# jiamiya/HOPE

Measured on AMD Instinct MI355X. Metric: parallel env steps/sec (full CarParking step incl. obs + RS search), higher is better.
Workload: dtype f64

## Files before the change

hope_amd/csrc/hope_internal.h:

```cpp
#pragma once
#include <hip/hip_runtime.h>
#include <stdint.h>
#include "hope_env.h"

namespace hope {

constexpr uint32_t STAGE_NO_BEAMS = 0x1000;
constexpr uint32_t STAGE_NO_MASK = 0x2000;
constexpr uint32_t STAGE_NO_CULL = 0x4000;
constexpr uint32_t STAGE_ONE_SCENE = 0x8000;

struct RsWord {
    double len[5];
    double Lm;
    int code;
    int n;
    double pad;
};
constexpr int RS_WORDS_PER_SCENE = 48;
constexpr int RS_LIST_MAX_SCENES = 1 << 24;
__host__ __device__ inline int rs_list_pack(int scene, int n_obst) { return (int)(((unsigned)scene << 8) | (unsigned)n_obst); }
__host__ __device__ inline int rs_list_scene(int entry) { return (int)((unsigned)entry >> 8); }
__host__ __device__ inline int rs_list_n_obst(int entry) { return (int)((unsigned)entry & 0xFFu); }
constexpr int RS_IN_WORDS = 14;
constexpr double RS_MAXC = 0.3327130214085973;
constexpr int RS_REC_HDR = 16;
constexpr int RS_REC_ORDER = 10;
constexpr int RS_REC_KEYS = RS_REC_HDR;
constexpr int RS_REC_WORDS = RS_REC_KEYS + RS_WORDS_PER_SCENE;
constexpr int RS_REC_SEGS = RS_REC_WORDS + 8 * RS_WORDS_PER_SCENE;
constexpr int RS_SEGW = 8, RS_SEG_F32 = 5 * RS_SEGW, RS_SEG_TABLE = RS_SEG_F32 + 5 * 2;
constexpr int RS_REC_DOUBLES = RS_REC_SEGS + RS_SEG_TABLE * RS_WORDS_PER_SCENE;

struct RsParams {
    int n, max_obst;
    int tile_cap;
    int max_queue;
    int slot_base, slot_dir;
    int obs_f64;
    int prio_front;
    const float4* obb;
    const float4* fverts;
    const float4* fbox;
    const uint8_t* eflag;
    const double* verts;
    const int32_t* n_obst;
    const double* scene_c;
    const double* state;
    const double* rs_in;
    const int32_t* rs_count;
    const int32_t* rs_list;
    double* rs_rec;
    int8_t* rs_word;
    void* rs_lengths;
    int32_t* surv_count;
    int2* surv_list;
};

struct DlpCases {
    int n_cases;
    const double* dest;
    const int32_t* cand_off;
    const double* cand;
    const int32_t* case_set;
    const int32_t* set_off;
    const double* set_verts;
};

struct StepCold {
    double* traj;
    int32_t* traj_len;
    int32_t* traj_valid;
    int32_t* layer_valid;
    const double* pool_verts;
    const double* pool_c;
    const int32_t* pool_nobst;
    const int32_t* pool_cls[2];
    int pool_cls_n[2];
    int32_t* cur_pool;
    uint32_t* episode;
    unsigned long long redraw_seed;
    DlpCases dlp;
    int32_t* pool_overflow;
    const uint8_t* slot_cls;
    float4* fverts;
    float4* fbox;
    uint8_t* eflag;
};

struct CwDev {
    unsigned long long* episodes;
    unsigned long long* successes;
    unsigned long long* folded_e;
    unsigned long long* folded_s;
    double* win_n;
    double* win_s;
    double* prob;
    double* pw;
};

constexpr int BEV_IMG = HOPE_IMG_SIZE;
constexpr int BEV_TRAJ_LEN = HOPE_TRAJ_RENDER_LEN;
constexpr int BEV_LAYER_ROWS = 512, BEV_LAYER_STRIDE = 128;
constexpr int BEV_DYN_DIM = 256;
constexpr size_t BEV_DYN_BYTES = (size_t)BEV_DYN_DIM * BEV_DYN_DIM;
constexpr int BEV_SCENE_INTS = 16 + (3 + BEV_TRAJ_LEN) * 16 + (2 + BEV_TRAJ_LEN) * 64;
struct BevParams {
    int n, max_obst;
    const double* verts;
    const int32_t* n_obst;
    const double* scene_c;
    const double* state;
    const double* traj;
    const int32_t* traj_len;
    int32_t* traj_valid;
    uint8_t* layer;
    uint8_t* dyn;
    int32_t* layer_valid;
    int32_t* legacy_list;
    int32_t* rebuild;
    int* scratch;
    const uint8_t* active;
    uint8_t* img;
    int debug;
};

struct LaunchTimer {
    virtual void begin(int kind, hipStream_t s) = 0;
    virtual void end(hipStream_t s) = 0;
};
hipError_t launch_rs_search(const RsParams& p, hipStream_t stream, LaunchTimer* timer);
hipError_t rs_prof_read(unsigned long long* out , int reset);
hipError_t rs_init_tables();
hipError_t rs_fstat_read(unsigned long long* out , int reset);
hipError_t rs_fdump_read(double* out );
hipError_t rs_log_read(int* out , int cap, int* n, int reset);
size_t rs_lds_bytes(int max_obst);
size_t rs_screen_lds_bytes(int max_obst);
size_t rs_rec_bytes_per_scene();
hipError_t launch_bev_image(const BevParams& p, hipStream_t stream, LaunchTimer* timer, hipStream_t side = nullptr, hipEvent_t ev_fork = nullptr,
                            hipEvent_t ev_join = nullptr);
size_t bev_lds_bytes(bool legacy);

}
```

hope_amd/csrc/hope_rs.hip:

```cpp
#include <stdlib.h>

#include "hope_dev.h"
#include "hope_internal.h"

namespace hope {

namespace {

constexpr double MAXC = RS_MAXC;
constexpr double RS_STEP = 0.1;
constexpr double MAX_LENGTH = 1000.0;
constexpr int NCAND = 46;

enum { TS = 0, TL = 1, TR = 2 };

__device__ __forceinline__ double py_mod(double v, double w) {
    double m = hm_fmod(v, w);
    if (m != 0) { if ((w < 0) != (m < 0)) m += w; } else m = copysign(0.0, w);
    return m;
}
__device__ __forceinline__ double rs_M(double theta) {
    double phi = py_mod(theta, 2.0 * PI);
    if (phi < -PI) phi += 2.0 * PI;
    if (phi > PI) phi -= 2.0 * PI;
// ... 347 lines not shown
        const double sp = (q == 1 || q == 2) ? -PHI : PHI;
        const double ssp = (q == 1 || q == 2) ? -sPHI : sPHI, csp = cPHI;
        double t = 0, u = 0, v = 0;
        bool ok = false;
        switch (g) {
            case 0: ok = (q == 0 || q == 2) && rs_SLS(sx, sy, sp, t, u, v); break;
            case 1: ok = rs_LSL(sx, sy, sp, ssp, csp, t, u, v); break;
            case 2: ok = rs_LSR(sx, sy, sp, ssp, csp, t, u, v); break;
            case 3: case 4: ok = rs_LRL(sx, sy, sp, ssp, csp, t, u, v); break;
            case 5: ok = rs_LRLRn(sx, sy, sp, ssp, csp, t, u, v); break;
            case 6: ok = rs_LRLRp(sx, sy, sp, ssp, csp, t, u, v); break;
            case 7: case 9: ok = rs_LRSL(sx, sy, sp, ssp, csp, t, u, v); break;
            case 8: case 10: ok = rs_LRSR(sx, sy, sp, ssp, csp, t, u, v); break;
            default: ok = rs_LRSLR(sx, sy, sp, ssp, csp, t, u, v); break;
        }
        ok = ok && live;
        int t0 = TL, t1 = TS, t2_ = TL, t3 = 0, t4 = 0, n = 3;
        double l0 = t, l1 = u, l2 = v, l3 = 0, l4 = 0;
        switch (g) {
            case 0: t0 = TS; t1 = TL; t2_ = TS; break;
            case 1: t0 = TL; t1 = TS; t2_ = TL; break;
            case 2: t0 = TL; t1 = TS; t2_ = TR; break;
            case 3: t0 = TL; t1 = TR; t2_ = TL; break;
            case 4: t0 = TL; t1 = TR; t2_ = TL; l0 = v; l2 = t; break;
            case 5: n = 4; t0 = TL; t1 = TR; t2_ = TL; t3 = TR; l2 = -u; l3 = v; break;
            case 6: n = 4; t0 = TL; t1 = TR; t2_ = TL; t3 = TR; l2 = u; l3 = v; break;
            case 7: n = 4; t0 = TL; t1 = TR; t2_ = TS; t3 = TL; l1 = -hp; l2 = u; l3 = v; break;
            case 8: n = 4; t0 = TL; t1 = TR; t2_ = TS; t3 = TR; l1 = -hp; l2 = u; l3 = v; break;
            case 9: n = 4; t0 = TL; t1 = TS; t2_ = TR; t3 = TL; l0 = v; l1 = u; l2 = -hp; l3 = t; break;
            case 10: n = 4; t0 = TR; t1 = TS; t2_ = TR; t3 = TL; l0 = v; l1 = u; l2 = -hp; l3 = t; break;
            default: n = 5; t0 = TL; t1 = TR; t2_ = TS; t3 = TL; t4 = TR; l1 = -hp; l2 = u; l3 = -hp; l4 = v; break;
        }
        if (q & 1) { l0 = -l0; l1 = -l1; l2 = -l2; l3 = -l3; l4 = -l4; }
        if (q & 2) { t0 = mirror_type(t0); t1 = mirror_type(t1); t2_ = mirror_type(t2_); t3 = mirror_type(t3); t4 = mirror_type(t4); }
        if (n < 4) { t3 = 0; l3 = 0; }
        if (n < 5) { t4 = 0; l4 = 0; }
        const int code = pack_types(t0, t1, t2_, t3, t4, n);
        double L = 0;
        L = L + fabs(l0); L = L + fabs(l1); L = L + fabs(l2);
        if (n > 3) L = L + fabs(l3);
        if (n > 4) L = L + fabs(l4);

        bool dup = false;
        if (g == 4 || g == 6) {
            const double a0 = (q & 2) ? quad_get<2>(p0) : quad_get<0>(p0), a1 = (q & 2) ? quad_get<2>(p1) : quad_get<0>(p1);
            const double a2 = (q & 2) ? quad_get<2>(p2) : quad_get<0>(p2), a3 = (q & 2) ? quad_get<2>(p3) : quad_get<0>(p3);
            const int ak = (q & 2) ? quad_get<2>((int)pk) : quad_get<0>((int)pk);
            const double b0 = (q & 2) ? quad_get<3>(p0) : quad_get<1>(p0), b1 = (q & 2) ? quad_get<3>(p1) : quad_get<1>(p1);
            const double b2 = (q & 2) ? quad_get<3>(p2) : quad_get<1>(p2), b3 = (q & 2) ? quad_get<3>(p3) : quad_get<1>(p3);
            const int bk = (q & 2) ? quad_get<3>((int)pk) : quad_get<1>((int)pk);
            dup = (ak && rs_dup(n, a0, a1, a2, a3, 0, l0, l1, l2, l3, l4)) || (bk && rs_dup(n, b0, b1, b2, b3, 0, l0, l1, l2, l3, l4));
        }
        bool kept = ok && !dup && !(L >= MAX_LENGTH) && !(q & 1);
        {
            const double e0 = (q & 2) ? quad_get<2>(l0) : quad_get<0>(l0), e1 = (q & 2) ? quad_get<2>(l1) : quad_get<0>(l1);
            const double e2 = (q & 2) ? quad_get<2>(l2) : quad_get<0>(l2), e3 = (q & 2) ? quad_get<2>(l3) : quad_get<0>(l3);
            const double e4 = (q & 2) ? quad_get<2>(l4) : quad_get<0>(l4);
            const int ek = (q & 2) ? quad_get<2>((int)kept) : quad_get<0>((int)kept);
            if (q & 1) kept = ok && !dup && !(ek && rs_dup(n, e0, e1, e2, e3, e4, l0, l1, l2, l3, l4)) && !(L >= MAX_LENGTH);
        }
        const double Lm = L / MAXC;
        if (live) rec[RS_REC_KEYS + 4 * g + q] = kept ? Lm : -1.0;
        if (kept) {
            RsWord* w = words + 4 * g + q;
            w->len[0] = l0; w->len[1] = l1; w->len[2] = l2; w->len[3] = l3; w->len[4] = l4;
            w->Lm = Lm; w->code = code; w->n = n;
        }
        p0 = l0; p1 = l1; p2 = l2; p3 = l3; pk = kept;
    }
}

__global__ __launch_bounds__(64) void k_rs_segs(RsParams p) {
    set_wave_prio(p.prio_front);
    __shared__ double keyl[8][RS_WORDS_PER_SCENE];
    __shared__ double prl[8][RS_WORDS_PER_SCENE];
    __shared__ unsigned char hidl[8][RS_WORDS_PER_SCENE];
    __shared__ unsigned char ordl[8][RS_WORDS_PER_SCENE];
    __shared__ int ntl[8];
    __shared__ double hdrl[8][8];
    const int lane = threadIdx.x, ls = lane >> 3, k0 = lane & 7;
    const int qi = blockIdx.x * 8 + ls;
    const int qs = qi < p.max_queue ? qi : p.max_queue - 1;
    const int entry = p.rs_list[qs];
    const int scene = rs_list_scene(entry);
    double* rec = p.rs_rec + (size_t)(p.slot_base + p.slot_dir * qs) * RS_REC_DOUBLES;
    const int count = *p.rs_count;
    if ((int)blockIdx.x * 8 >= count) return;
    const bool live = qi < count;
    double keyv[RS_WORDS_PER_SCENE / 8];
#pragma unroll
    for (int j = 0; j < RS_WORDS_PER_SCENE / 8; j++) keyv[j] = live ? rec[RS_REC_KEYS + 8 * j + k0] : -1.0;
    const double* in = p.rs_in + (size_t)qs * RS_IN_WORDS;
    double hdr = 0.0;
    int hdr_n = 0;
    if (k0 < 3) hdr = in[k0];
    else if (k0 < 7) hdr = in[k0];
    else hdr_n = rs_list_n_obst(entry);
    unsigned long long keptm = 0;
#pragma unroll
    for (int j = 0; j < RS_WORDS_PER_SCENE / 8; j++) {
        const double key = live ? keyv[j] : -1.0;
        keyl[ls][8 * j + k0] = key;
        keptm |= ((__ballot(key >= 0.0) >> (8 * ls)) & 0xffull) << (8 * j);
    }
    __syncthreads();
    if (live && k0 == 0) {
        double* pr = prl[ls];
        unsigned char* hid = hidl[ls];
        int hn = 0;
        for (unsigned long long m = keptm; m; m &= m - 1) {
            const int c = __ffsll((long long)m) - 1;
            const double pv = keyl[ls][c];
            int i = hn++;
            pr[i] = pv; hid[i] = (unsigned char)c;
            while (i) {
                const int parent = (i - 1) >> 1;
                if (pr[parent] < pr[i]) break;
                const double tp = pr[i]; pr[i] = pr[parent]; pr[parent] = tp;
                const unsigned char ti = hid[i]; hid[i] = hid[parent]; hid[parent] = ti;
                i = parent;
            }
        }
        const int n_kept = hn;
        int no = 0;
        double lmin = 0;
        while (hn > 0) {
            const double lm = pr[0];
            if (no == 0) lmin = lm;
            if (lm > 1.6 * lmin && no + 1 > 2) break;
            ordl[ls][no++] = hid[0];
            if (hn == 1) { hn = 0; break; }
            hn--;
            pr[0] = pr[hn]; hid[0] = hid[hn];
            int i = 0;
            for (;;) {
                const int l = (i << 1) + 1, r = (i + 1) << 1;
                int low = (l < hn && pr[l] < pr[i]) ? l : i;
                if (r < hn && pr[r] < pr[low]) low = r;
                if (low == i) break;
                const double tp = pr[i]; pr[i] = pr[low]; pr[low] = tp;
                const unsigned char ti = hid[i]; hid[i] = hid[low]; hid[low] = ti;
                i = low;
            }
        }
        ntl[ls] = no;
        ((int2*)rec)[1] = make_int2(n_kept, no);
    }
    if (live) {
        if (k0 < 7) rec[2 + k0] = hdr;
        else ((int2*)rec)[0] = make_int2(scene, hdr_n);
        hdrl[ls][k0] = hdr;
    }
    __syncthreads();
    if (!live) return;
    const int n_test = ntl[ls];
    const unsigned char* order = ordl[ls];
    const double q0w = hdrl[ls][2];
    double sq0, cq0;
    hm_sincos(q0w, &sq0, &cq0);
    const double fq0x = hdrl[ls][0] - hdrl[ls][3], fq0y = hdrl[ls][1] - hdrl[ls][5];
    for (int k = k0; k < n_test; k += 8) {
        const double* W = rec + RS_REC_WORDS + 8 * (int)order[k];
        double len[5];
#pragma unroll
        for (int i = 0; i < 5; i++) len[i] = W[i];
        const double w6 = W[6];
        const int code = __double2loint(w6), nseg = __double2hiint(w6);
        double* tb = rec + RS_REC_SEGS + RS_SEG_TABLE * k;
        double ox = 0, oy = 0, hy = 0;
#pragma unroll
        for (int i = 0; i < 5; i++) {
            if (i < nseg) {
                const int m = type_of(code, i);
                const double l = len[i];
                double s_oy, c_oy;
                hm_sincos(hy, &s_oy, &c_oy);
                double* sp_ = tb + RS_SEGW * i;
                sp_[0] = ox; sp_[1] = oy; sp_[2] = hy; sp_[3] = c_oy; sp_[4] = s_oy; sp_[5] = (double)m; sp_[6] = l;
                if (i == 0) sp_[7] = w6;
                {
// ... 506 lines not shown
    const double r0 = lane < RS_REC_HDR ? rec[lane] : 0.0;
    const double* tables = rec + RS_REC_SEGS;
    {
        typedef __attribute__((address_space(3))) void* lds_ptr;
        const double2* t2 = (const double2*)tables;
        __builtin_amdgcn_global_load_lds((const void*)(t2 + lane), (lds_ptr)tabs, 16, 0, 0);
        if (lane < 2 * RS_SEG_TABLE - WAVE) __builtin_amdgcn_global_load_lds((const void*)(t2 + WAVE + lane), (lds_ptr)(tabs + 2 * WAVE), 16, 0, 0);
        const float4* gfv = p.fverts + (size_t)scene * p.max_obst * 2;
        const float4* gfb = p.fbox + (size_t)scene * p.max_obst;
        const uint32_t* gfl = (const uint32_t*)(p.eflag + (size_t)scene * eflag_stride(p.max_obst));
        float4* lfv = (float4*)fv;
        for (int base = 0; base < 2 * n_obst; base += WAVE)
            if (base + lane < 2 * n_obst) __builtin_amdgcn_global_load_lds((const void*)(gfv + base + lane), (lds_ptr)(lfv + base), 16, 0, 0);
        for (int base = 0; base < n_obst; base += WAVE)
            if (base + lane < n_obst) __builtin_amdgcn_global_load_lds((const void*)(gfb + base + lane), (lds_ptr)(fbox + base), 16, 0, 0);
        for (int base = 0; 4 * base < n_obst; base += WAVE)
            if (4 * (base + lane) < n_obst) __builtin_amdgcn_global_load_lds((const void*)(gfl + base + lane), (lds_ptr)((uint32_t*)eflag + base), 4, 0, 0);
    }
    asm volatile("s_waitcnt vmcnt(0)" ::: "memory");
    const int n_paths = __builtin_amdgcn_readlane(__double2hiint(r0), 1);
    if (n_paths == 0) return;
    const float fxmax = (float)(readlane_d(r0, 6) - readlane_d(r0, 5)), fymax = (float)(readlane_d(r0, 8) - readlane_d(r0, 7));
    lsync();
    const unsigned long long condemned = screen_words<TIMING>(lane, n_paths, n_obst, tables, tabs, pq, cand, fv, fbox, eflag, fxmax, fymax, tsec);
    if (lane == 0) {
        ((unsigned long long*)rec)[9] = condemned;
        if (condemned != ((1ull << n_paths) - 1)) p.surv_list[atomicAdd(p.surv_count, 1)] = make_int2(qidx, entry);
    }
}

template <int OCC, bool TIMING, bool STATS, bool PRE = false>
__global__ __launch_bounds__(64, OCC) void k_rs_validate_f(RsParams p, int obs_f64) {
    extern __shared__ __attribute__((aligned(16))) double lds[];
    const int lane = threadIdx.x;
    if (!(obs_f64 & 0x10000)) __builtin_amdgcn_s_setprio(1);
    unsigned long long tsec[16] = {};
    const unsigned long long tstart_ = TIMING ? __builtin_readcyclecounter() : 0;
    RS_T0();
    const int b_ = (int)blockIdx.x;
    int qidx, entry;
    if (PRE) {
        const int2 sv = p.surv_list[b_];
        if (b_ >= *p.surv_count) return;
        qidx = sv.x; entry = sv.y;
    } else {
#ifdef HOPE_RS_3TRIPS
        const int count = *p.rs_count;
        if (b_ >= count) return;
        qidx = scene_of_block(b_, count);
        entry = p.rs_list[qidx];
#else
        qidx = scene_of_block(b_, p.max_queue);
        entry = p.rs_list[qidx];
        const int count = *p.rs_count;
        if (qidx >= count) return;
#endif
    }
    const int slot = p.slot_base + p.slot_dir * qidx;
#ifndef HOPE_RS_HDR
    const int scene = rs_list_scene(entry);
    const int n_obst = rs_list_n_obst(entry);
#endif
    float2* fv = (float2*)lds;
    float4* fbox = (float4*)(lds + 4 * p.tile_cap);
    double* scr = lds + 6 * p.tile_cap;
    double* segp = scr + RSB_SEG;
    double* qpd = scr + RSB_QPD;
    int* cand = (int*)(scr + RSB_WORDS_F);
    double* tabl = scr + RSB_TABF;
    unsigned char* qseg = (unsigned char*)(cand + ((p.tile_cap + 3) & ~3));
    unsigned char* eflag = qseg + RSB_QCAP;

    const double* rec = p.rs_rec + (size_t)slot * RS_REC_DOUBLES;
    const double r0 = lane < RS_REC_HDR ? rec[lane] : 0.0;
    const double* tables = rec + RS_REC_SEGS;
#ifdef HOPE_RS_3TRIPS
    if (__builtin_amdgcn_readlane(__double2hiint(r0), 1) == 0) return;
#endif
#ifdef HOPE_RS_HDR
    const int scene = __builtin_amdgcn_readlane(__double2loint(r0), 0);
    const int n_obst = __builtin_amdgcn_readlane(__double2hiint(r0), 0);
    (void)entry;
#endif
    double tb = lane < RS_SEG_TABLE ? tables[lane] : 0.0;
    if (!PRE) {
        typedef __attribute__((address_space(3))) void* lds_ptr;
        const double2* t2 = (const double2*)tables;
        __builtin_amdgcn_global_load_lds((const void*)(t2 + lane), (lds_ptr)qpd, 16, 0, 0);
        if (lane < 2 * RS_SEG_TABLE - WAVE) __builtin_amdgcn_global_load_lds((const void*)(t2 + WAVE + lane), (lds_ptr)(qpd + 2 * WAVE), 16, 0, 0);
    }
    {
        typedef __attribute__((address_space(3))) void* lds_ptr;
        const float4* gfv = p.fverts + (size_t)scene * p.max_obst * 2;
        const float4* gfb = p.fbox + (size_t)scene * p.max_obst;
        const uint32_t* gfl = (const uint32_t*)(p.eflag + (size_t)scene * eflag_stride(p.max_obst));
        float4* lfv = (float4*)fv;
        for (int base = 0; base < 2 * n_obst; base += WAVE)
            if (base + lane < 2 * n_obst) __builtin_amdgcn_global_load_lds((const void*)(gfv + base + lane), (lds_ptr)(lfv + base), 16, 0, 0);
        for (int base = 0; base < n_obst; base += WAVE)
            if (base + lane < n_obst) __builtin_amdgcn_global_load_lds((const void*)(gfb + base + lane), (lds_ptr)(fbox + base), 16, 0, 0);
        for (int base = 0; 4 * base < n_obst; base += WAVE)
            if (4 * (base + lane) < n_obst) __builtin_amdgcn_global_load_lds((const void*)(gfl + base + lane), (lds_ptr)((uint32_t*)eflag + base), 4, 0, 0);
    }
    const int n_paths = __builtin_amdgcn_readlane(__double2hiint(r0), 1);
    if (n_paths == 0) {
        asm volatile("s_waitcnt vmcnt(0)" ::: "memory");
        return;
    }
    const double* verts_g = p.verts + (size_t)scene * p.max_obst * 8;
    const float fxmin = 0.0f, fxmax = (float)(readlane_d(r0, 6) - readlane_d(r0, 5)), fymin = 0.0f, fymax = (float)(readlane_d(r0, 8) - readlane_d(r0, 7));
    const double step = RS_STEP * MAXC;
    bool tile_pending = true;
    int found = -1;
    double* bad1 = scr + RSB_BAD;
    if (lane < 6) bad1[lane] = INFINITY;
    lsync();
    RS_T(0);
    const bool paranoid = (obs_f64 & 0x2000) != 0;
    unsigned long long st_pass = 0, st_hit = 0, st_exact = 0, st_unc = 0, st_bad_hit = 0, st_bad_clear = 0, st_samples = 0;
    unsigned long long st_why[5] = {};
    unsigned long long condemned = 0;
    if (PRE) condemned = (unsigned long long)__double_as_longlong(readlane_d(r0, 9));
    else if (!(obs_f64 & 0x20000)) {
        asm volatile("s_waitcnt vmcnt(0)" ::: "memory");
        tile_pending = false;
        condemned = screen_words<TIMING>(lane, n_paths, n_obst, tables, qpd, (int*)tabl ,
                                         cand, fv, fbox, eflag, fxmax, fymax, tsec);
        if (TIMING) t0_ = __builtin_readcyclecounter();
    }
    else {
        asm volatile("s_waitcnt vmcnt(0)" ::: "memory");
        tile_pending = false;
    }
    const bool verify_screen = STATS && paranoid;
    const bool all_condemned = condemned == ((1ull << n_paths) - 1);
    unsigned long long st_scr_words = __popcll(condemned), st_scr_dead = all_condemned ? 1 : 0, st_scr_bad = 0;
    if (!all_condemned || verify_screen) {
        const double T0 = g_rs_steps[lane], T1 = g_rs_steps[WAVE + lane], T2 = g_rs_steps[2 * WAVE + lane], T3 = g_rs_steps[3 * WAVE + lane];
        tabl[lane] = T0; tabl[WAVE + lane] = T1; tabl[2 * WAVE + lane] = T2; tabl[3 * WAVE + lane] = T3;
        lsync();
    }
    for (int idx = 1; idx <= n_paths; idx++) {
        if (all_condemned && !verify_screen) break;
        const double tcur = tb;
        if (idx < n_paths && lane < RS_SEG_TABLE) tb = tables[RS_SEG_TABLE * idx + lane];
        const double len0 = readlane_d(tcur, 6), w6 = readlane_d(tcur, 7);
        const int code = __double2loint(w6), nseg = __double2hiint(w6);
        const int cls1 = type_of(code, 0) * 2 + (len0 > 0.0 ? 1 : 0);
        if (bad1[cls1] > 0.0 && fabs(len0) >= bad1[cls1]) continue;
        const bool screened = (condemned >> (idx - 1)) & 1;
        if (screened && !verify_screen) continue;
        bool invalid = false;
        if (lane < RS_SEG_TABLE) segp[lane] = tcur;
        if (TIMING) tsec[9] += 1;
        {
            double zero;
            asm volatile("v_mov_b64 %0, 0" : "=v"(zero));
            if (lane == 0) { qpd[0] = zero; qseg[0] = (unsigned char)__double2loint(zero); }
        }
        int nq = 1;
        lsync();
        RS_T(1);
        const int win = 128;
        int i = 0, t_off = 0;
        bool seg_open = false, finished = false;
        double pd = 0, ll = 0.0, lprev = 0.0, d = 0, l = 0;
        while (!invalid && (!finished || nq > 0)) {
            while (!finished && nq + WAVE + 1 <= win) {
                if (TIMING) tsec[10] += 1;
                if (!seg_open) {
                    l = uni_d(segp[RSB_SEGW * i + 6]);
                    d = uni_d(l > 0.0 ? step : -step);
                    pd = uni_d((i >= 1 && (lprev * l) > 0) ? -d - ll : d - ll);
                    lprev = l;
                    seg_open = true;
                }
                double mine, t = pd;
                int ncap;
                if (i == 0 && t_off + WAVE <= RS_TAB) {
                    const double v = tabl[t_off + lane];
                    mine = d > 0.0 ? v : -v;
                    ncap = WAVE;
                    t_off += WAVE;
                    if (t_off < RS_TAB) {
                        const double nx = tabl[t_off];
                        t = d > 0.0 ? nx : -nx;
                    } else t = readlane_d(mine, WAVE - 1) + d;
                } else {
                    mine = pd;
                    double last = pd;
                    ncap = 0;
                    for (int j0 = 0; j0 < WAVE; j0 += 8) {
                        if ((lane >> 3) == (j0 >> 3)) mine = t;
#pragma unroll
                        for (int jj = 0; jj < 7; jj++) t = t + d;
                        last = t;
                        t = t + d;
                        ncap = j0 + 8;
                        if (__any(fabs(last) > fabs(l))) break;
                    }
#pragma unroll
                    for (int k = 0; k < 7; k++)
                        if (k < (lane & 7)) mine = mine + d;
                }
                const bool in_seg = lane < ncap && fabs(mine) <= fabs(l);
                const unsigned long long valid = (ncap == WAVE) ? ~0ull : ((1ull << ncap) - 1);
                const unsigned long long fail = ~__ballot(in_seg) & valid;
                const int cnt = fail ? (__ffsll((long long)fail) - 1) : ncap;
                if (lane < cnt) { qpd[nq + lane] = mine; qseg[nq + lane] = (unsigned char)i; }
                nq += cnt;
                if (fail) {
                    pd = readlane_d(mine, cnt);
                    ll = uni_d(l - pd - d);
                    seg_open = false;
                    if (i == nseg - 1) {
                        if (lane == 0) { qpd[nq] = l; qseg[nq] = (unsigned char)i; }
                        nq += 1;
                        finished = true;
                    }
                    i++;
                } else pd = uni_d(t);
            }
            lsync();
            RS_T(2);
            if (finished && segp[3 * RSB_SEGW + 7] != 0.0) nq = pop_trailing_zero_x(nq, segp, RSB_SEGW, qpd, qseg, lane);
            const int n_all = nq;
            const int n = finished ? n_all : (n_all & ~(WAVE - 1));
            const int stride = (n + WAVE - 1) >> 6;
            const int n_coarse = stride == 1 ? n : (stride == 2 ? (n + 1) >> 1 : ((n + 2) * 171) >> 9);
            const int n_rest = n - n_coarse;
            for (int rnd = 0; rnd == 0 || (rnd - 1) * WAVE < n_rest; rnd++) {
                int sidx;
                if (rnd == 0) sidx = (lane < n_coarse) ? stride * lane : -1;
                else { const int r = (rnd - 1) * WAVE + lane; sidx = r < n_rest ? r + (stride == 2 ? r : r >> 1) + 1 : -1; }
                const bool active = sidx >= 0;
                if (TIMING) tsec[11] += 1;
                float X = 0, Y = 0, hc = 1, hs = 0;
                int sg0 = 0;
                if (active) {
                    const float lf = (float)qpd[sidx];
                    sg0 = (int)qseg[sidx];
                    const float4 row = ((const float4*)(segp + RS_SEG_F32))[sg0];
                    const int m = type_of(code, sg0);
                    const float rev = lf * 0.15915494309189535f;
                    const float sl = m == TS ? 0.0f : __builtin_amdgcn_sinf(rev), cl = m == TS ? 1.0f : __builtin_amdgcn_cosf(rev);
                    const float sgn = m == TR ? -1.0f : 1.0f;
                    const float ldx = m == TS ? lf * F_INV_MAXC : sl * F_INV_MAXC;
                    const float ldy = sgn * (1.0f - cl) * F_INV_MAXC;
                    X = row.x + (row.z * ldx - row.w * ldy);
                    Y = row.y + (row.w * ldx + row.z * ldy);
                    const float ss = sgn * sl;
                    hc = row.z * cl - row.w * ss;
                    hs = row.w * cl + row.z * ss;
                }
                RS_T(3);
                int why_cnt = 0, hit_rec = -1;
                int ua = -1, ub = -1;
                bool uover = false;
                bool hit = active && (X < fxmin - FEPS || X > fxmax + FEPS || Y < fymin - FEPS || Y > fymax + FEPS);
                bool unc = active && !hit && (X < fxmin + FEPS || X > fxmax - FEPS || Y < fymin + FEPS || Y > fymax - FEPS);
                const float cx = X + hc * F_MID, cy = Y + hs * F_MID;
                const float ex = fabsf(hc) * F_HL + fabsf(hs) * F_HW + FEPS, ey = fabsf(hs) * F_HL + fabsf(hc) * F_HW + FEPS;
                const float lox = cx - ex, hix = cx + ex, loy = cy - ey, hiy = cy + ey;
                const float ulox = wave_min_f(active ? lox : INFINITY), uhix = wave_max_f(active ? hix : -INFINITY);
                const float uloy = wave_min_f(active ? loy : INFINITY), uhiy = wave_max_f(active ? hiy : -INFINITY);
                if (tile_pending) {
                    asm volatile("s_waitcnt vmcnt(0)" ::: "memory");
                    tile_pending = false;
                }
                int nc = 0;
                for (int base = 0; base < n_obst; base += WAVE) {
                    const int o = base + lane;
                    bool near = false;
                    if (o < n_obst) {
                        const float4 bb = fbox[o];
                        near = !(bb.x > uhix || bb.y < ulox || bb.z > uhiy || bb.w < uloy);
                    }
                    const unsigned long long mm = __ballot(near);
                    if (near) cand[nc + __popcll(mm & ((1ull << lane) - 1))] = o;
                    nc += __popcll(mm);
                }
                RS_T(4);
                if (nc > 0 && !__any(hit)) {
                    if (TIMING) { tsec[12] += 1; tsec[13] += nc; }
                    lsync();
                    const bool hull_ok = fminf(fabsf(hc), fabsf(hs)) >= FETA_HULL;
// ... 49 lines not shown
                            const bool certain = cross && corners_ok && angle_ok && hull_ok && ((efl >> k) & 1);
                            const bool mine_open = (open >> k) & 1;
                            if (mine_open && certain) { hit = true; if (STATS && hit_rec < 0) hit_rec = r * 4 + k; }
                            if (STATS && mine_open && !certain) why_cnt |= 1 << (!cross ? 0 : !((efl >> k) & 1) ? 1 : !hull_ok ? 2 : !corners_ok ? 3 : 4);
                            if (!__any(hit) && mine_open && !certain) {
                                unc = true;
                                if (ua < 0) ua = r | (0x100 << k);
                                else if ((ua & 0xff) == r) ua |= 0x100 << k;
                                else if (ub < 0) ub = r | (0x100 << k);
                                else if ((ub & 0xff) == r) ub |= 0x100 << k;
                                else uover = true;
                            }
                        }
                        if (__any(hit)) break;
                    }
                    lsync();
                }
                RS_T(5);
                bool bad = hit;
                const bool any_hit = __any(hit);
                const bool need64 = (STATS && paranoid) || (!any_hit && __any(unc));
                (void)need64;
                if (STATS) {
                    st_pass += 1;
                    if (any_hit) st_hit += 1;
                    if (!any_hit && __any(unc)) {
                        const unsigned long long wm = __ballot(why_cnt != 0);
                        int wor = 0;
                        for (int b = 0; b < 5; b++) if (__any((why_cnt >> b) & 1)) wor |= 1 << b;
                        for (int b = 0; b < 5; b++) st_why[b] += (wor >> b) & 1;
                        (void)wm;
                    }
                }
                if (STATS && paranoid) {
                    const double q0x = rec[2], q0y = rec[3], q0w = rec[4], xmin = rec[5], xmax = rec[6], ymin = rec[7], ymax = rec[8];
                    const double c_q = rec[RS_REC_SEGS + RS_SEGW + 7], s_q = rec[RS_REC_SEGS + 2 * RS_SEGW + 7];
                    const bool ex = exact_pass<true>(active ? sidx : -1, segp, qpd, qseg, c_q, s_q, q0x, q0y, q0w, verts_g, p.obb + (size_t)scene * p.max_obst, cand, n_obst, xmin, xmax, ymin, ymax, lane);
                    st_samples += __popcll(__ballot(active));
                    st_bad_hit += __popcll(__ballot(active && hit && !ex));
                    if (active && ((hit && !ex) || (!any_hit && !hit && !unc && ex))) {
                        const int di = (int)atomicAdd(&g_rs_fstat[15], 1ull);
                        if (di < 64) {
                            double px = 0, py = 0, pyaw = 0;
                            const double spd = qpd[sidx];
                            const double* sp_ = segp + RSB_SEGW * (int)qseg[sidx];
                            interpolate(spd, (int)sp_[5], sp_[0], sp_[1], sp_[2], sp_[3], -sp_[4], sp_[3], sp_[4], px, py, pyaw);
                            const double wyaw = pi_2_pi(pyaw + q0w);
                            double* dd = g_rs_fdump + 16 * di;
                            dd[0] = scene; dd[1] = idx; dd[2] = spd; dd[3] = (double)qseg[sidx]; dd[4] = X; dd[5] = Y; dd[6] = hc; dd[7] = hs;
                            dd[8] = c_q * px + s_q * py; dd[9] = -s_q * px + c_q * py; dd[10] = hm_cos(wyaw); dd[11] = hm_sin(wyaw);
                            dd[12] = hit ? 1.0 : 0.0; dd[13] = (double)why_cnt; dd[14] = sp_[5]; dd[15] = (double)hit_rec;
                        }
                    }
                    if (!any_hit) st_bad_clear += __popcll(__ballot(active && !hit && !unc && ex));
                    bad = ex;
                } else if (!any_hit && __any(unc)) {
                    if (STATS) { st_exact += 1; st_unc += __popcll(__ballot(unc)); }
                    bad = exact_edges(unc, sidx, ua, ub, uover, cand, nc, segp, qpd, qseg, verts_g, rec);
                }
                if (TIMING) t0_ = __builtin_readcyclecounter();
                if (__any(bad)) {
                    const double mine1 = (bad && active && qseg[sidx] == 0) ? fabs(qpd[sidx]) : INFINITY;
                    const double v = fmin(bad1[cls1], wave_min_d(mine1));
                    lsync();
                    if (lane < 6 && (lane == cls1 || v == 0.0)) bad1[lane] = fmin(bad1[lane], v);
                    invalid = true;
                    break;
                }
            }
            {
                const int rem = n_all - n;
                double cd = 0;
                unsigned char cs = 0;
                if (lane < rem) { cd = qpd[n + lane]; cs = qseg[n + lane]; }
                lsync();
                if (lane < rem) { qpd[lane] = cd; qseg[lane] = cs; }
                nq = rem;
            }
            lsync();
        }
        if (STATS && screened && !invalid) { st_scr_bad += 1; continue; }
        if (!invalid) { found = idx - 1; break; }
    }
    if (STATS && lane == 0) {
        atomicAdd(&g_rs_fstat[7], st_scr_bad); atomicAdd(&g_rs_fstat[13], st_scr_words); atomicAdd(&g_rs_fstat[14], st_scr_dead);
        for (int b = 0; b < 5; b++) atomicAdd(&g_rs_fstat[8 + b], st_why[b]);
        atomicAdd(&g_rs_fstat[0], st_pass); atomicAdd(&g_rs_fstat[1], st_hit); atomicAdd(&g_rs_fstat[2], st_exact);
        atomicAdd(&g_rs_fstat[3], st_unc); atomicAdd(&g_rs_fstat[4], st_bad_hit); atomicAdd(&g_rs_fstat[5], st_bad_clear);
        atomicAdd(&g_rs_fstat[6], st_samples);
    }
    if (TIMING) {
        tsec[6] = __builtin_readcyclecounter() - tstart_;
        tsec[8] = 1;
        if (lane == 0) {
            for (int i = 0; i < 16; i++) if (tsec[i]) atomicAdd(&g_rs_prof[(blockIdx.x & 63) * 16 + i], tsec[i]);
            const int li = atomicAdd(&g_rs_log_n, 1);
            if (li < RS_LOG_CAP) g_rs_log[li] = make_int4((int)tsec[6], (int)tsec[9] | (n_paths << 8) | ((p.tile_cap > 32) << 16), (int)tsec[11], found >= 0);
        }
    }
    if (found < 0) return;
    const double wlen = lane < 5 ? segp[RSB_SEGW * lane + 6] : 0.0;
    const int code = __double2loint(segp[7]), nseg = __double2hiint(segp[7]);
    if (lane < 5) {
        double lm = lane < nseg ? wlen / MAXC : 0.0;
        if (p.rs_lengths) {
            if (obs_f64 & 1) ((double*)p.rs_lengths)[5 * (size_t)scene + lane] = lm;
            else ((float*)p.rs_lengths)[5 * (size_t)scene + lane] = (float)lm;
        }
        p.rs_word[8 * (size_t)scene + lane] = lane < nseg ? (int8_t)type_of(code, lane) : (int8_t)HOPE_RS_NONE;
    }
    if (lane == 5) p.rs_word[8 * (size_t)scene + 5] = (int8_t)nseg;
    if (lane == 6) p.rs_word[8 * (size_t)scene + 6] = 1;
}

}

static size_t rs_lds_bytes_exact(int max_obst) {
    return (size_t)(10 * max_obst + RSB_WORDS) * 8 + (size_t)((max_obst + 3) & ~3) * 4 + RSB_QCAP;
}
static size_t rs_lds_bytes_filter(int max_obst) {
    return (size_t)(6 * max_obst + RSB_WORDS_F) * 8 + (size_t)((max_obst + 3) & ~3) * 4 + RSB_QCAP + (size_t)((max_obst + 3) & ~3);
}
size_t rs_lds_bytes(int max_obst) { return std::max(rs_lds_bytes_exact(max_obst), rs_lds_bytes_filter(max_obst)); }
size_t rs_screen_lds_bytes(int max_obst) {
    return (size_t)(6 * max_obst + 4 * RS_SEG_TABLE) * 8 + 2 * WAVE * 4 + (size_t)((max_obst + 3) & ~3) * 4 + (size_t)((max_obst + 3) & ~3);
}
size_t rs_rec_bytes_per_scene() { return sizeof(double) * RS_REC_DOUBLES; }

hipError_t rs_prof_read(unsigned long long* out, int reset) {
    hipError_t e = hipDeviceSynchronize();
    if (e != hipSuccess) return e;
    static unsigned long long buf[64 * 16];
    e = hipMemcpyFromSymbol(buf, HIP_SYMBOL(g_rs_prof), sizeof(buf));
    for (int i = 0; i < 16; i++) { out[i] = 0; for (int sh = 0; sh < 64; sh++) out[i] += buf[sh * 16 + i]; }
    if (e == hipSuccess && reset) {
        for (auto& v : buf) v = 0;
        e = hipMemcpyToSymbol(HIP_SYMBOL(g_rs_prof), buf, sizeof(buf));
    }
    return e;
}

hipError_t rs_fdump_read(double* out ) {
    hipError_t e = hipDeviceSynchronize();
    if (e != hipSuccess) return e;
    return hipMemcpyFromSymbol(out, HIP_SYMBOL(g_rs_fdump), sizeof(double) * 64 * 16);
}

hipError_t rs_log_read(int* out , int cap, int* n, int reset) {
    hipError_t e = hipDeviceSynchronize();
    if (e != hipSuccess) return e;
    e = hipMemcpyFromSymbol(n, HIP_SYMBOL(g_rs_log_n), sizeof(int));
    if (e != hipSuccess) return e;
    const int m = *n < cap ? (*n < RS_LOG_CAP ? *n : RS_LOG_CAP) : cap;
    if (m > 0) e = hipMemcpyFromSymbol(out, HIP_SYMBOL(g_rs_log), sizeof(int4) * (size_t)m);
    if (e == hipSuccess && reset) { const int z = 0; e = hipMemcpyToSymbol(HIP_SYMBOL(g_rs_log_n), &z, sizeof(int)); }
    return e;
}

hipError_t rs_fstat_read(unsigned long long* out , int reset) {
    hipError_t e = hipDeviceSynchronize();
    if (e != hipSuccess) return e;
    e = hipMemcpyFromSymbol(out, HIP_SYMBOL(g_rs_fstat), 16 * sizeof(unsigned long long));
    if (e == hipSuccess && reset) {
        unsigned long long z[16] = {};
        e = hipMemcpyToSymbol(HIP_SYMBOL(g_rs_fstat), z, sizeof(z));
    }
    return e;
}

hipError_t rs_init_tables() {
    static bool done[64] = {};
    int dev = 0;
    hipError_t e = hipGetDevice(&dev);
    if (e != hipSuccess) return e;
    if (dev >= 0 && dev < 64 && done[dev]) return hipSuccess;
    double tab[RS_TAB];
    const volatile double step = RS_STEP * MAXC;
    volatile double t = step;
    for (int k = 0; k < RS_TAB; k++) { tab[k] = t; t = t + step; }
    e = hipMemcpyToSymbol(HIP_SYMBOL(g_rs_steps), tab, sizeof(tab));
    if (e == hipSuccess && dev >= 0 && dev < 64) done[dev] = true;
    return e;
}

constexpr int RS_LARGE_TILE_WPC = 6;
constexpr int RS_PRIO_MIN_SCENES = 32768;

hipError_t launch_rs_search(const RsParams& p, hipStream_t stream, LaunchTimer* timer) {
    if (p.max_queue <= 0) return hipSuccess;
    static const bool timing = getenv("HOPE_RS_TIMING") != nullptr;
    const bool exact = getenv("HOPE_RS_EXACT") != nullptr;
    const int dbg = getenv("HOPE_RS_DEBUG") ? (int)strtol(getenv("HOPE_RS_DEBUG"), nullptr, 0) : 0;
    const bool stats = (dbg & 0x6000) != 0;
    size_t lds = exact ? rs_lds_bytes_exact(p.tile_cap) : rs_lds_bytes_filter(p.tile_cap);
    if (!exact && p.tile_cap > 32) lds = std::max(lds, (size_t)((158 * 1024 / RS_LARGE_TILE_WPC) & ~255));
    if (lds > 48 * 1024) {
        hipError_t e = hipFuncSetAttribute((const void*)k_rs_validate_f<RSF_OCC, false, false, true>, hipFuncAttributeMaxDynamicSharedMemorySize, (int)lds);
        if (e != hipSuccess) return e;
    }
    const void* vk = exact ? (timing ? (const void*)k_rs_validate<3, true> : (const void*)k_rs_validate<3, false>)
                           : (timing ? (const void*)k_rs_validate_f<RSF_OCC, true, false> : stats ? (const void*)k_rs_validate_f<RSF_OCC, false, true>
                              : (const void*)k_rs_validate_f<RSF_OCC, false, false>);
    if (lds > 48 * 1024) {
        hipError_t e = hipFuncSetAttribute(vk, hipFuncAttributeMaxDynamicSharedMemorySize, (int)lds);
        if (e != hipSuccess) return e;
    }
    if (!exact) { hipError_t e = rs_init_tables(); if (e != hipSuccess) return e; }
    if (timer) timer->begin(HOPE_K_RS_WORDS, stream);
    hipLaunchKernelGGL(k_rs_words, dim3((p.max_queue + RSA_SCENES - 1) / RSA_SCENES, RSA_GROUPS), dim3(WAVE), 0, stream, p);
    if (timer) timer->end(stream);
    if (timer) timer->begin(HOPE_K_RS_SEGS, stream);
    hipLaunchKernelGGL(k_rs_segs, dim3((p.max_queue + 7) / 8), dim3(WAVE), 0, stream, p);
    if (timer) timer->end(stream);
    const bool split = !exact && !timing && !stats && !(dbg & 0x20000) && p.surv_count && p.surv_list &&
                       getenv("HOPE_RS_SPLIT") && atoi(getenv("HOPE_RS_SPLIT")) == 1;
    if (split) {
        if (timer) timer->begin(HOPE_K_RS_SCREEN, stream);
        hipLaunchKernelGGL((k_rs_screen<false, 8>), dim3(p.max_queue), dim3(WAVE), rs_screen_lds_bytes(p.tile_cap), stream, p);
        if (timer) timer->end(stream);
    }
    if (timer) timer->begin(HOPE_K_RS_VALIDATE, stream);
    const bool longer_chain = 2 * (long long)p.max_queue >= p.n;
    const int flags = (p.obs_f64 ? 1 : 0) | dbg | ((p.n < RS_PRIO_MIN_SCENES || !longer_chain) ? 0x10000 : 0);
    if (exact) {
        if (timing) hipLaunchKernelGGL((k_rs_validate<3, true>), dim3(p.max_queue), dim3(WAVE), lds, stream, p, flags);
        else hipLaunchKernelGGL((k_rs_validate<3, false>), dim3(p.max_queue), dim3(WAVE), lds, stream, p, flags);
    } else if (split) hipLaunchKernelGGL((k_rs_validate_f<RSF_OCC, false, false, true>), dim3(p.max_queue), dim3(WAVE), lds, stream, p, flags);
    else if (timing) hipLaunchKernelGGL((k_rs_validate_f<RSF_OCC, true, false>), dim3(p.max_queue), dim3(WAVE), lds, stream, p, flags);
    else if (stats) hipLaunchKernelGGL((k_rs_validate_f<RSF_OCC, false, true>), dim3(p.max_queue), dim3(WAVE), lds, stream, p, flags);
    else hipLaunchKernelGGL((k_rs_validate_f<RSF_OCC, false, false>), dim3(p.max_queue), dim3(WAVE), lds, stream, p, flags);
    if (timer) timer->end(stream);
    return hipGetLastError();
}

}
```

Measured before the change: 162.0 million.

## Async-load RS step table into LDS and skip condemned words in validate

The validate kernel now iterates only over non-condemned candidate words using a bitmask instead of scanning every index. It stages the step table into LDS with asynchronous global_load_lds, waiting on vmcnt only when the table is first needed. The segs kernel issues its key and input loads before the early-exit check to overlap latency. An optional env-gated path syncs the stream to shrink the validate grid to the live count.

```diff
diff --git a/hope_amd/csrc/hope_internal.h b/hope_amd/csrc/hope_internal.h
--- a/hope_amd/csrc/hope_internal.h
+++ b/hope_amd/csrc/hope_internal.h
@@ -55,6 +55,7 @@
     void* rs_lengths;
     int32_t* surv_count;
     int2* surv_list;
+    const double* rs_steps = nullptr;
 };
 
 struct DlpCases {
@@ -131,7 +132,7 @@
 };
 hipError_t launch_rs_search(const RsParams& p, hipStream_t stream, LaunchTimer* timer);
 hipError_t rs_prof_read(unsigned long long* out , int reset);
-hipError_t rs_init_tables();
+hipError_t rs_init_tables(const double** steps = nullptr);
 hipError_t rs_fstat_read(unsigned long long* out , int reset);
 hipError_t rs_fdump_read(double* out );
 hipError_t rs_log_read(int* out , int cap, int* n, int reset);
diff --git a/hope_amd/csrc/hope_rs.hip b/hope_amd/csrc/hope_rs.hip
--- a/hope_amd/csrc/hope_rs.hip
+++ b/hope_amd/csrc/hope_rs.hip
@@ -453,20 +453,18 @@
     const int qi = blockIdx.x * 8 + ls;
     const int qs = qi < p.max_queue ? qi : p.max_queue - 1;
     const int entry = p.rs_list[qs];
-    const int scene = rs_list_scene(entry);
     double* rec = p.rs_rec + (size_t)(p.slot_base + p.slot_dir * qs) * RS_REC_DOUBLES;
+    double keyv[RS_WORDS_PER_SCENE / 8];
+#pragma unroll
+    for (int j = 0; j < RS_WORDS_PER_SCENE / 8; j++) keyv[j] = rec[RS_REC_KEYS + 8 * j + k0];
+    const double* in = p.rs_in + (size_t)qs * RS_IN_WORDS;
+    const double hdr_in = in[k0 < 7 ? k0 : 0];
     const int count = *p.rs_count;
     if ((int)blockIdx.x * 8 >= count) return;
     const bool live = qi < count;
-    double keyv[RS_WORDS_PER_SCENE / 8];
-#pragma unroll
-    for (int j = 0; j < RS_WORDS_PER_SCENE / 8; j++) keyv[j] = live ? rec[RS_REC_KEYS + 8 * j + k0] : -1.0;
-    const double* in = p.rs_in + (size_t)qs * RS_IN_WORDS;
-    double hdr = 0.0;
-    int hdr_n = 0;
-    if (k0 < 3) hdr = in[k0];
-    else if (k0 < 7) hdr = in[k0];
-    else hdr_n = rs_list_n_obst(entry);
+    const int scene = rs_list_scene(entry);
+    const double hdr = k0 < 7 ? hdr_in : 0.0;
+    const int hdr_n = k0 < 7 ? 0 : rs_list_n_obst(entry);
     unsigned long long keptm = 0;
 #pragma unroll
     for (int j = 0; j < RS_WORDS_PER_SCENE / 8; j++) {
@@ -1139,8 +1137,9 @@
     const int n_obst = __builtin_amdgcn_readlane(__double2hiint(r0), 0);
     (void)entry;
 #endif
-    double tb = lane < RS_SEG_TABLE ? tables[lane] : 0.0;
-    if (!PRE) {
+    double tb = 0.0;
+    if (PRE) { if (lane < RS_SEG_TABLE) tb = tables[lane]; }
+    else {
         typedef __attribute__((address_space(3))) void* lds_ptr;
         const double2* t2 = (const double2*)tables;
         __builtin_amdgcn_global_load_lds((const void*)(t2 + lane), (lds_ptr)qpd, 16, 0, 0);
@@ -1192,21 +1191,33 @@
     const bool verify_screen = STATS && paranoid;
     const bool all_condemned = condemned == ((1ull << n_paths) - 1);
     unsigned long long st_scr_words = __popcll(condemned), st_scr_dead = all_condemned ? 1 : 0, st_scr_bad = 0;
-    if (!all_condemned || verify_screen) {
-        const double T0 = g_rs_steps[lane], T1 = g_rs_steps[WAVE + lane], T2 = g_rs_steps[2 * WAVE + lane], T3 = g_rs_steps[3 * WAVE + lane];
-        tabl[lane] = T0; tabl[WAVE + lane] = T1; tabl[2 * WAVE + lane] = T2; tabl[3 * WAVE + lane] = T3;
+    unsigned long long todo = verify_screen ? (1ull << n_paths) - 1 : ((1ull << n_paths) - 1) & ~condemned;
+    bool tab_ready = false;
+    if (todo) {
+        const int k = __ffsll((long long)todo) - 1;
+        const int lk = PRE ? -1 : k - ((obs_f64 & 0x20000) ? 0 : ((n_paths - 1) & ~3));
+        if (!PRE && lk >= 0) { if (lane < RS_SEG_TABLE) tb = qpd[RS_SEG_TABLE * lk + lane]; }
+        else if (!PRE || k > 0) { if (lane < RS_SEG_TABLE) tb = tables[RS_SEG_TABLE * k + lane]; }
+        typedef __attribute__((address_space(3))) void* lds_ptr;
+        const double2* s2 = (const double2*)p.rs_steps;
         lsync();
-    }
-    for (int idx = 1; idx <= n_paths; idx++) {
-        if (all_condemned && !verify_screen) break;
+        __builtin_amdgcn_global_load_lds((const void*)(s2 + lane), (lds_ptr)tabl, 16, 0, 0);
+        __builtin_amdgcn_global_load_lds((const void*)(s2 + WAVE + lane), (lds_ptr)(tabl + 2 * WAVE), 16, 0, 0);
+    }
+    for (bool first_word = true; todo; first_word = false) {
+        const int idx = __ffsll((long long)todo);
+        todo &= todo - 1;
+        if (!first_word) {
+            asm volatile("s_waitcnt vmcnt(0)" ::: "memory");
+            tab_ready = true;
+        }
         const double tcur = tb;
-        if (idx < n_paths && lane < RS_SEG_TABLE) tb = tables[RS_SEG_TABLE * idx + lane];
+        if (todo && lane < RS_SEG_TABLE) tb = tables[RS_SEG_TABLE * (__ffsll((long long)todo) - 1) + lane];
         const double len0 = readlane_d(tcur, 6), w6 = readlane_d(tcur, 7);
         const int code = __double2loint(w6), nseg = __double2hiint(w6);
         const int cls1 = type_of(code, 0) * 2 + (len0 > 0.0 ? 1 : 0);
         if (bad1[cls1] > 0.0 && fabs(len0) >= bad1[cls1]) continue;
         const bool screened = (condemned >> (idx - 1)) & 1;
-        if (screened && !verify_screen) continue;
         bool invalid = false;
         if (lane < RS_SEG_TABLE) segp[lane] = tcur;
         if (TIMING) tsec[9] += 1;
@@ -1234,7 +1245,11 @@
                 }
                 double mine, t = pd;
                 int ncap;
-                if (i == 0 && t_off + WAVE <= RS_TAB) {
+                if (i == 0 && (tab_ready || t_off > 0) && t_off + WAVE <= RS_TAB) {
+                    if (!tab_ready) {
+                        asm volatile("s_waitcnt vmcnt(0)" ::: "memory");
+                        tab_ready = true;
+                    }
                     const double v = tabl[t_off + lane];
                     mine = d > 0.0 ? v : -v;
                     ncap = WAVE;
@@ -1259,6 +1274,7 @@
 #pragma unroll
                     for (int k = 0; k < 7; k++)
                         if (k < (lane & 7)) mine = mine + d;
+                    if (i == 0) t_off += WAVE;
                 }
                 const bool in_seg = lane < ncap && fabs(mine) <= fabs(l);
                 const unsigned long long valid = (ncap == WAVE) ? ~0ull : ((1ull << ncap) - 1);
@@ -1474,6 +1490,7 @@
         if (STATS && screened && !invalid) { st_scr_bad += 1; continue; }
         if (!invalid) { found = idx - 1; break; }
     }
+    asm volatile("s_waitcnt vmcnt(0)" ::: "memory");
     if (STATS && lane == 0) {
         atomicAdd(&g_rs_fstat[7], st_scr_bad); atomicAdd(&g_rs_fstat[13], st_scr_words); atomicAdd(&g_rs_fstat[14], st_scr_dead);
         for (int b = 0; b < 5; b++) atomicAdd(&g_rs_fstat[8 + b], st_why[b]);
@@ -1560,26 +1577,31 @@
     return e;
 }
 
-hipError_t rs_init_tables() {
+hipError_t rs_init_tables(const double** steps) {
     static bool done[64] = {};
+    static const double* addr[64] = {};
     int dev = 0;
     hipError_t e = hipGetDevice(&dev);
     if (e != hipSuccess) return e;
-    if (dev >= 0 && dev < 64 && done[dev]) return hipSuccess;
+    if (dev >= 0 && dev < 64 && done[dev]) { if (steps) *steps = addr[dev]; return hipSuccess; }
     double tab[RS_TAB];
     const volatile double step = RS_STEP * MAXC;
     volatile double t = step;
     for (int k = 0; k < RS_TAB; k++) { tab[k] = t; t = t + step; }
     e = hipMemcpyToSymbol(HIP_SYMBOL(g_rs_steps), tab, sizeof(tab));
-    if (e == hipSuccess && dev >= 0 && dev < 64) done[dev] = true;
+    void* a = nullptr;
+    if (e == hipSuccess) e = hipGetSymbolAddress(&a, HIP_SYMBOL(g_rs_steps));
+    if (e == hipSuccess && dev >= 0 && dev < 64) { done[dev] = true; addr[dev] = (const double*)a; }
+    if (e == hipSuccess && steps) *steps = (const double*)a;
     return e;
 }
 
 constexpr int RS_LARGE_TILE_WPC = 6;
 constexpr int RS_PRIO_MIN_SCENES = 32768;
 
-hipError_t launch_rs_search(const RsParams& p, hipStream_t stream, LaunchTimer* timer) {
-    if (p.max_queue <= 0) return hipSuccess;
+hipError_t launch_rs_search(const RsParams& p_, hipStream_t stream, LaunchTimer* timer) {
+    if (p_.max_queue <= 0) return hipSuccess;
+    RsParams p = p_;
     static const bool timing = getenv("HOPE_RS_TIMING") != nullptr;
     const bool exact = getenv("HOPE_RS_EXACT") != nullptr;
     const int dbg = getenv("HOPE_RS_DEBUG") ? (int)strtol(getenv("HOPE_RS_DEBUG"), nullptr, 0) : 0;
@@ -1597,7 +1619,8 @@
         hipError_t e = hipFuncSetAttribute(vk, hipFuncAttributeMaxDynamicSharedMemorySize, (int)lds);
         if (e != hipSuccess) return e;
     }
-    if (!exact) { hipError_t e = rs_init_tables(); if (e != hipSuccess) return e; }
+    p.rs_steps = nullptr;
+    if (!exact) { hipError_t e = rs_init_tables(&p.rs_steps); if (e != hipSuccess) return e; }
     if (timer) timer->begin(HOPE_K_RS_WORDS, stream);
     hipLaunchKernelGGL(k_rs_words, dim3((p.max_queue + RSA_SCENES - 1) / RSA_SCENES, RSA_GROUPS), dim3(WAVE), 0, stream, p);
     if (timer) timer->end(stream);
@@ -1611,6 +1634,14 @@
         hipLaunchKernelGGL((k_rs_screen<false, 8>), dim3(p.max_queue), dim3(WAVE), rs_screen_lds_bytes(p.tile_cap), stream, p);
         if (timer) timer->end(stream);
     }
+    RsParams pv = p;
+    if (!exact && !split && getenv("HOPE_RS_CUT_GRID")) {
+        int c = 0;
+        hipError_t e = hipStreamSynchronize(stream);
+        if (e == hipSuccess) e = hipMemcpy(&c, p.rs_count, sizeof(int), hipMemcpyDeviceToHost);
+        if (e != hipSuccess) return e;
+        pv.max_queue = std::min(std::max(c, 1), p.max_queue);
+    }
     if (timer) timer->begin(HOPE_K_RS_VALIDATE, stream);
     const bool longer_chain = 2 * (long long)p.max_queue >= p.n;
     const int flags = (p.obs_f64 ? 1 : 0) | dbg | ((p.n < RS_PRIO_MIN_SCENES || !longer_chain) ? 0x10000 : 0);
@@ -1618,9 +1649,9 @@
         if (timing) hipLaunchKernelGGL((k_rs_validate<3, true>), dim3(p.max_queue), dim3(WAVE), lds, stream, p, flags);
         else hipLaunchKernelGGL((k_rs_validate<3, false>), dim3(p.max_queue), dim3(WAVE), lds, stream, p, flags);
     } else if (split) hipLaunchKernelGGL((k_rs_validate_f<RSF_OCC, false, false, true>), dim3(p.max_queue), dim3(WAVE), lds, stream, p, flags);
-    else if (timing) hipLaunchKernelGGL((k_rs_validate_f<RSF_OCC, true, false>), dim3(p.max_queue), dim3(WAVE), lds, stream, p, flags);
-    else if (stats) hipLaunchKernelGGL((k_rs_validate_f<RSF_OCC, false, true>), dim3(p.max_queue), dim3(WAVE), lds, stream, p, flags);
-    else hipLaunchKernelGGL((k_rs_validate_f<RSF_OCC, false, false>), dim3(p.max_queue), dim3(WAVE), lds, stream, p, flags);
+    else if (timing) hipLaunchKernelGGL((k_rs_validate_f<RSF_OCC, true, false>), dim3(pv.max_queue), dim3(WAVE), lds, stream, pv, flags);
+    else if (stats) hipLaunchKernelGGL((k_rs_validate_f<RSF_OCC, false, true>), dim3(pv.max_queue), dim3(WAVE), lds, stream, pv, flags);
+    else hipLaunchKernelGGL((k_rs_validate_f<RSF_OCC, false, false>), dim3(pv.max_queue), dim3(WAVE), lds, stream, pv, flags);
     if (timer) timer->end(stream);
     return hipGetLastError();
 }
```

Measured after the change: 162.5 million (median of 3 runs). Within noise of the previous version (+0.3%).
